# mfkiwl/conan-slam

Measured on AMD Instinct MI355X. Metric: ekf_update_steps_per_sec, higher is better.
Workload: dtype f32

## Files before the change

conan_slam_amd/csrc/cslam_ekf.hip:

```cpp
#include <hip/hip_runtime.h>

#include <algorithm>
#include <atomic>
#include <cfloat>
#include <cmath>
#include <cstdint>
#include <cstdlib>
#include <new>
#include <string>
#include <thread>
#include <vector>

#include "cslam_common.hpp"
#include "device_owners.hpp"
#include "ekf_kernels.hpp"
#include "ekf_kernels_fast.hpp"
#include "ekf_landmark_kernels.hpp"
#include "ekf_lookahead.hpp"
#include "ekf_pgemm_limbs.hpp"
#include "ekf_pose_kernels.hpp"
#include "host_linalg.hpp"

namespace cslam
{
__global__ void ekf_la_signal_kernel(unsigned* signal, unsigned add)
{
    if (threadIdx.x == 0)
    {
        atomicAdd(signal, add);
    }
}
__global__ void __launch_bounds__(128) ekf_la_wide_f32(LaWideArgs a)
{
    ekf_la_wide_body<1, 0>(a);
}
__global__ void __launch_bounds__(128) ekf_la_wide_f32_k64(LaWideArgs a)
{
    ekf_la_wide_body<1, 64>(a);
}
}

using namespace cslam;

namespace
{

std::atomic<int>& g_engines = ::cslam::live_engines();

constexpr int    kStagingSlots = 64;
constexpr size_t kLdsBudget    = 150 * 1024;

struct EkfBase
{
    virtual ~EkfBase() {}
    int         dtype    = CSLAM_F32;
    int         fuse_f64 = 1;
    int         pgemm_limbs_req = -1, limbs_kmin_req = -1;
    int         xcd_queues_req = -1;
    int         device   = 0;
    int         quirks   = CSLAM_Q_REF_EXACT;
    int         nmax     = 0;
    int         ncap     = 0;
    int         ldp      = 0;
    int         n        = 3;
    int         sync_mode = 1;
    int         seq_defer     = 1;
    int         lower         = 0;
    int         pipeline      = 0;
    int         pgemm_spare   = 16;
    int         gather_corr_wide = 1;
    int         pgemm_wgs     = 0;
    int         lookahead     = -1;
    Stream      stream_own, stream_b_own, stream_f_own;
    hipStream_t stream   = nullptr;
    hipStream_t stream_b = nullptr;
    long long   la_windows = 0;

    virtual int init()                                                                        = 0;
    virtual int set_state(const void* X, int n, const void* P, int ldp)                        = 0;
    virtual int get_state(void* X, void* P, int ldp)                                           = 0;
    virtual int get_x(void* X, int cap)                                                        = 0;
    virtual int get_landmarks(int first, int count, void* x, void* pll, void* pvl)             = 0;
    virtual int trace(double* tr)                                                              = 0;
    virtual int predict(double v, double swa, const void* Q, double wb, double dt)             = 0;
    virtual int update(const void* Z, int m, const void* R, const int* idf, int batch, bool on_device) = 0;
    virtual int augment(const void* Z, int q, const void* R)                                   = 0;
    virtual int observe_heading(double phi, int use)                                           = 0;
    virtual int associate(const void* Z, int m, const void* R, double g1, double g2, int* idf_out, int* kind) = 0;
    virtual int factor_status(int* flags, int clear)                                           = 0;
    virtual int set_profiling(int on)                                                          = 0;
    virtual int get_stage_times(double* ms, int* launches)                                     = 0;
    virtual int debug_last_update(void* PHT, void* S, void* G, void* W1, void* V, int* k)      = 0;
    virtual int set_deferred(int max_cols)                                                     = 0;
    virtual int do_flush()                                                                     = 0;
    virtual int resolve_predict()                                                              = 0;
    virtual void set_fuse_predict(int on)                                                      = 0;
    virtual int sync_all()                                                                     = 0;
    virtual int la_drain()                                                                     = 0;
};

template <typename T>
struct Ekf : EkfBase
{
    DevBuf<T>   dX, dP;
    DevBuf<T>   dPv;
    DevBuf<int> dPoseDone;
    DevBuf<int> dSign;
    DevBuf<T>   dLm;
    int  hd_cols[2] = {0, 0};
// ... 42 lines not shown
    DevBuf<unsigned char>    dStage;
    Event                    stage_ev[kStagingSlots];
    int         stage_next = 0;
    DevBuf<int> dTicket;
    int        pgemm_limbs = 0;
    int        xcd_queues  = 0;
    int        limbs_kmin  = 65;
    DevBuf<uint4> dWb;
    size_t        wb_bytes = 0;
    DevBuf<int2>  dTilesM;
    DevBuf<int>   dSegOff;
    DevBuf<int>   dTicketX;
    int        tilesM_built = 0;
    int        limb_parity = 0;
    unsigned   launch_parity = 0;
    int        psym_nt = -1;
    DevBuf<int2> dTiles;
    int   tiles_built = 0;
    int   n_sym_tiles = 0;
    int   num_cus     = 256;
    int sticky_host = 0;
    int last_k      = 0;
    int kp_call_limit = 0;
    int                     profiling = 0;
    unsigned                prof_count = 0;
    bool                    prof_sampled = false;
    std::vector<Event>      ev_pool;
    std::vector<int>        ev_stage;
    size_t                  ev_used = 0;

    ~Ekf() override
    {
        (void)hipSetDevice(device);
        if (stream)
        {
            (void)hipStreamSynchronize(stream);
        }
        if (stream_b && stream_b != stream)
        {
            (void)hipStreamSynchronize(stream_b);
        }
        if (stream_f)
        {
            (void)hipStreamSynchronize(stream_f);
        }
    }

    T* wbase(int region) const { return dW1.get() + (size_t)region * wcap * ldp; }

    int use_device() { CSLAM_HIP_TRY(hipSetDevice(device)); return CSLAM_OK; }

    int init() override
    {
        int rc = use_device();
        if (rc)
        {
            return rc;
        }
        if (xcd_queues_req >= 0)
        {
            xcd_queues = xcd_queues_req;
        }
        if (pgemm_limbs_req >= 0)
        {
            pgemm_limbs = (pgemm_limbs_req == 6 || pgemm_limbs_req == 9) ? pgemm_limbs_req : 0;
        }
// ... 30 lines not shown
        if ((rc = dX.alloc_zeroed((size_t)ldp, stream)) || (rc = dP.alloc_zeroed((size_t)ldp * ldp, stream)) ||
            (rc = dPv.alloc_zeroed((size_t)3 * ldp, stream)) || (rc = dPoseDone.alloc_zeroed(4, stream)) ||
            (rc = dFlags.alloc_zeroed(2, stream)) || (rc = hFlags.alloc(2)) ||
            (rc = dHead.alloc_zeroed((size_t)3 * ldp + 2, stream)))
        {
            return rc;
        }
        CSLAM_HIP_TRY(hipFuncSetAttribute(reinterpret_cast<const void*>(&ekf_factor_kernel<T>),
                                          hipFuncAttributeMaxDynamicSharedMemorySize, 160 * 1024));
        if (sizeof(T) == 4)
        {
            CSLAM_HIP_TRY(hipFuncSetAttribute(reinterpret_cast<const void*>(&ekf_factor_mfma_big_f32<128>),
                                              hipFuncAttributeMaxDynamicSharedMemorySize, 160 * 1024));
        }
        else
        {
            CSLAM_HIP_TRY(hipFuncSetAttribute(reinterpret_cast<const void*>(&ekf_factor_mfma_f64<64>),
                                              hipFuncAttributeMaxDynamicSharedMemorySize, 160 * 1024));
            CSLAM_HIP_TRY(hipFuncSetAttribute(reinterpret_cast<const void*>(&ekf_factor_mfma_f64<32>),
                                              hipFuncAttributeMaxDynamicSharedMemorySize, 160 * 1024));
            CSLAM_HIP_TRY(hipFuncSetAttribute(reinterpret_cast<const void*>(&ekf_downdate_f64<4>),
                                              hipFuncAttributeMaxDynamicSharedMemorySize, 160 * 1024));
            CSLAM_HIP_TRY(hipFuncSetAttribute(reinterpret_cast<const void*>(&ekf_downdate_f64<2>),
                                              hipFuncAttributeMaxDynamicSharedMemorySize, 160 * 1024));
        }
        CSLAM_TRY(dTicket.alloc_zeroed(2, stream));
        if (const char* sv = getenv("CSLAM_LA_K64"))
        {
            la_k64 = atoi(sv) ? 1 : 0;
        }
        if (const char* sv = getenv("CSLAM_LA_WG_SIGNAL"))
        {
            la_wg_signal = atoi(sv) ? 1 : 0;
        }
        if (const char* sv = getenv("CSLAM_PSYM_NT"))
        {
            psym_nt = atoi(sv) ? 1 : 0;
        }
        rc = ensure_k(64);
        if (rc)
        {
            return rc;
        }
        rc = ensure_w(128);
        if (rc)
        {
            return rc;
        }
        rc = ensure_m(64);
        if (rc)
        {
            return rc;
        }
        CSLAM_HIP_TRY(hipStreamSynchronize(stream));
        return CSLAM_OK;
    }

    int ensure_k(int k)
    {
        if (k <= kcap)
        {
            return CSLAM_OK;
        }
        int newk = round_up(std::max(k, 2 * kcap), 8);
        CSLAM_HIP_TRY(hipStreamSynchronize(stream));
        Workspace nw;
// ... 189 lines not shown
    {
        return sizeof(T) == 4 && (k8 <= 128 || limbs_take(k8)) && lower && ldp < 32768;
    }
    bool limbs_take(int k8) const
    {
        return sizeof(T) == 4 && pgemm_limbs > 0 && k8 >= limbs_kmin && k8 <= 256 && lower && ldp < 32768;
    }

    int launch_negcol_fix(T* W, int kcols, hipStream_t st)
    {
        const int tiles = round_up(n, kTile) / kTile;
        int       rc    = CSLAM_OK;
        if (lower && (rc = ensure_tile_list(tiles)))
        {
            return rc;
        }
        const int nt = lower ? n_sym_tiles : tiles * tiles;
        hipLaunchKernelGGL(ekf_negcol_fix_kernel<T>, dim3(std::min(nt, 2 * num_cus)), dim3(256), 0, st, dP.get(), ldp,
                           n, W, ldp, kcols, dSign.get() + (size_t)wcur * wcap, dSign.get() + (size_t)2 * wcap + wcur,
                           lower ? dTiles.get() : (const int2*)nullptr, nt, tiles, dPoseDone.get() + 2,
                           (stream_b == stream) ? 1 : 0);
        CSLAM_HIP_TRY(hipGetLastError());
        return CSLAM_OK;
    }

    int flush_wait()
    {
        int rc = flush();
        return rc ? rc : wait_pgemm();
    }

    size_t slot_bytes(int mc) const { return (size_t)mc * (2 * sizeof(T) + sizeof(int)); }

    int ensure_m(int m)
    {
        if (m <= mcap)
        {
            return CSLAM_OK;
        }
        int newm = std::max(m, 2 * mcap);
        if (int rc = la_drain())
        {
            return rc;
        }
        CSLAM_HIP_TRY(hipStreamSynchronize(stream));
        if (stream_f)
        {
            CSLAM_HIP_TRY(hipStreamSynchronize(stream_f));
        }
        PinnedBuf<unsigned char> hs;
        DevBuf<unsigned char>    ds;
        int                      rc = hs.alloc(slot_bytes(newm) * kStagingSlots);
        if (rc || (rc = ds.alloc(slot_bytes(newm) * kStagingSlots)))
        {
            return rc;
        }
        hStage = std::move(hs);
        dStage = std::move(ds);
        mcap = newm;
        return CSLAM_OK;
    }

    int stage_obs(const void* Z, const int* idf, int m, bool on_device, const T** dZ, const int** dIdf)
    {
        int rc = ensure_m(m);
        if (rc)
        {
            return rc;
        }
        int slot = stage_next;
        stage_next = (stage_next + 1) % kStagingSlots;
        if (stage_ev[slot])
        {
            CSLAM_HIP_TRY(hipEventSynchronize(stage_ev[slot].get()));
        }
        else if ((rc = stage_ev[slot].create(hipEventDisableTiming)))
        {
            return rc;
        }
        size_t         zb = (size_t)m * 2 * sizeof(T);
        unsigned char* ds = dStage.get() + slot_bytes(mcap) * slot;
        if (on_device)
        {
            hipLaunchKernelGGL(ekf_stage_obs_kernel<T>, dim3((3 * m + 255) / 256), dim3(256), 0, stream,
                               static_cast<const T*>(Z), idf, m, reinterpret_cast<T*>(ds), reinterpret_cast<int*>(ds + zb));
            CSLAM_HIP_TRY(hipGetLastError());
        }
        else
        {
            unsigned char* hs = hStage.get() + slot_bytes(mcap) * slot;
            memcpy(hs, Z, zb);
            memcpy(hs + zb, idf, (size_t)m * sizeof(int));
            CSLAM_HIP_TRY(hipMemcpyAsync(ds, hs, zb + (size_t)m * sizeof(int), hipMemcpyHostToDevice, stream));
        }
        CSLAM_HIP_TRY(hipEventRecord(stage_ev[slot].get(), stream));
        *dZ   = reinterpret_cast<const T*>(ds);
        *dIdf = reinterpret_cast<const int*>(ds + zb);
        return CSLAM_OK;
    }

    int set_state(const void* X, int nn, const void* P, int ldph) override
    {
        if (!X || !P || nn < 3 || nn > ncap || ((nn - 3) & 1) || ldph < nn)
        {
            return fail(CSLAM_ERR_BAD_ARG, "set_state: bad n=%d (cap %d) or ldp=%d", nn, ncap, ldph);
        }
        int rc = sync_all();
        if (rc)
        {
            return rc;
        }
        CSLAM_HIP_TRY(hipMemcpyAsync(dX.get(), X, (size_t)nn * sizeof(T), hipMemcpyHostToDevice, stream));
        CSLAM_HIP_TRY(hipMemcpy2DAsync(dP.get(), (size_t)ldp * sizeof(T), P, (size_t)ldph * sizeof(T),
                                       (size_t)nn * sizeof(T), (size_t)nn, hipMemcpyHostToDevice, stream));
        CSLAM_HIP_TRY(hipMemcpyAsync(dPv.get(), dP.get(), (size_t)3 * ldp * sizeof(T), hipMemcpyDeviceToDevice,
                                     stream));
        kp        = 0;
        wcur      = 0;
        last_slot = nullptr;
// ... 714 lines not shown
            if ((rc = launch_downdate(last_slot, k, stream)))
            {
                return rc;
            }
        }
        CSLAM_HIP_TRY(hipStreamSynchronize(stream));
        return CSLAM_OK;
    }


    struct LaUpd
    {
        const T*       dZ;
        const int*     dIdf;
        int            m;
        T              R[4];
        PredictArgs<T> pp;
    };
    struct FactorOut
    {
        DevBuf<T>   S, G, Gt, V, t, U, M, sub, xloc;
        DevBuf<int> idloc;
    };
    struct LaSet
    {
        Event          ev_fb;
        Event          ev_raw;
        FactorOut      fo[2];
        DevBuf<T>      XL, PvL, PH, PvLb, Dbb;
        DevBuf<T>      Y;
        DevBuf<LaModel<T>> model;
        DevBuf<unsigned>   done;
        DevBuf<long long>  stamps;
    };
    LaUpd       la_q[2];
    int         la_n = 0;
    LaSet       la;
    bool        la_ready = false;
    hipStream_t stream_f = nullptr;
    DevBuf<T>   la_WR;
    int         la_kpad  = 0;
    int         la_cus = 0;
    unsigned    la_target = 0;
    unsigned    la_seq    = 0;
    unsigned    la_sig_add = 0;
    int         la_k64 = 1;
    int         la_wg_signal = 0;

    int         la_fused   = 1;
    const T *dbgS = nullptr, *dbgGt = nullptr, *dbgV = nullptr;

    int la_ensure(int kp_cols)
    {
        constexpr int KM = 2 * kLaMaxObs;
        if (!la_ready)
        {
            int lo = 0, hi = 0;
            CSLAM_HIP_TRY(hipDeviceGetStreamPriorityRange(&lo, &hi));
            Stream sf;
            LaSet  nl;
            int    rc = sf.create_with_priority(hipStreamNonBlocking, hi);
            if (rc || (rc = nl.ev_fb.create(hipEventDisableTiming)) || (rc = nl.ev_raw.create(hipEventDisableTiming)))
            {
                return rc;
            }
            CSLAM_HIP_TRY(hipFuncSetAttribute(reinterpret_cast<const void*>(&ekf_la_chain_kernel<T, 32>),
                                              hipFuncAttributeMaxDynamicSharedMemorySize, (int)la_chain_lds<T>(32)));
            CSLAM_HIP_TRY(hipFuncSetAttribute(reinterpret_cast<const void*>(&ekf_la_chain_kernel<T, 64>),
                                              hipFuncAttributeMaxDynamicSharedMemorySize, (int)la_chain_lds<T>(64)));
            CSLAM_TRY(nl.done.alloc_zeroed_blocking(768));
            for (FactorOut& f : nl.fo)
            {
                const size_t kk = (size_t)KM * (KM + 1);
                if ((rc = f.S.alloc(kk)) || (rc = f.G.alloc(kk)) || (rc = f.Gt.alloc(kk)) || (rc = f.V.alloc(KM)) ||
                    (rc = f.t.alloc(KM)) || (rc = f.U.alloc(KM)) || (rc = f.M.alloc((size_t)3 * KM)) ||
                    (rc = f.sub.alloc((size_t)(3 + KM) * KM)) || (rc = f.xloc.alloc(3 + KM)) ||
                    (rc = f.idloc.alloc(kLaMaxObs)))
                {
                    return rc;
                }
            }
            if ((rc = nl.XL.alloc((size_t)2 * KM)) || (rc = nl.PvL.alloc((size_t)2 * KM * 3)) ||
                (rc = nl.PH.alloc((size_t)KM * KM)) || (rc = nl.PvLb.alloc((size_t)KM * 3)) ||
                (rc = nl.Dbb.alloc((size_t)KM * KM)) || (rc = nl.Y.alloc((size_t)KM * KM)) ||
                (rc = nl.model.alloc(2)) || (getenv("CSLAM_LA_STAMPS") && (rc = nl.stamps.alloc_zeroed_blocking(32))))
            {
                return rc;
            }
            if (const char* fv = getenv("CSLAM_LA_FUSED"))
            {
                la_fused = atoi(fv) ? 1 : 0;
            }
            stream_f_own = std::move(sf);
            stream_f     = stream_f_own.get();
            la           = std::move(nl);
            la_cus       = 1;
            la_target    = 0;
            la_seq       = 0;
            la_ready     = true;
        }
        if (kp_cols > la_kpad)
        {
            CSLAM_HIP_TRY(hipStreamSynchronize(stream));
            CSLAM_HIP_TRY(hipStreamSynchronize(stream_f));
            const int kpad = round_up(std::max(kp_cols, 128), 64);
            DevBuf<T> wr;
            CSLAM_TRY(wr.alloc((size_t)2 * KM * kpad));
            la_WR   = std::move(wr);
            la_kpad = kpad;
        }
        return CSLAM_OK;
    }

    bool la_eligible(int m) const
    {
        const int k = 2 * m;
        const bool on = lookahead > 0 || (lookahead < 0 && sizeof(T) == 4 && n >= 7000 && g_engines.load() == 1);
        return on && !sync_mode && !pipeline && profiling != 1 && k > 16 && k <= 2 * kLaMaxObs && gather_corr_wide &&
               fuse_predict && (sizeof(T) == 4 || fuse_f64) && defer_max >= k + (la_n ? 2 * la_q[0].m : k) &&
               wcap >= k + (la_n ? 2 * la_q[0].m : k) && seq.count == 0 && hd_cols[0] == 0 && hd_cols[1] == 0 && n > 3 &&
               kp_call_limit == 0;
    }

    int la_enqueue(const T* dZ, const int* dIdf, int m, const T* R, bool on_device)
    {
        if (on_device && la_n == 0)
        {
            if (int rc = stage_obs(dZ, dIdf, m, true, &dZ, &dIdf))
            {
                return rc;
            }
        }
        LaUpd u;
        u.dZ   = dZ;
        u.dIdf = dIdf;
        u.m    = m;
        for (int i = 0; i < 4; i++)
        {
            u.R[i] = R[i];
        }
        u.pp     = pp;
        pp.valid = 0;
        la_q[la_n++] = u;
        return la_n == 2 ? la_launch_window() : CSLAM_OK;
    }

    FactorArgs<T> la_factor_args(const LaUpd& u, FactorOut& f)
    {
        FactorArgs<T> a;
        a.X   = f.xloc.get();
        a.n   = 3 + 2 * u.m;
        a.Z   = u.dZ;
        a.idf = la.fo[0].idloc.get();
        a.m   = u.m;
        for (int i = 0; i < 4; i++)
        {
            a.R[i] = u.R[i];
        }
        a.PHT      = ws.dPHT.get();
        a.ldw      = ldp;
        a.dS       = f.S.get();
        a.dG       = f.G.get();
        a.dGt      = f.Gt.get();
        a.dV       = f.V.get();
        a.dt       = f.t.get();
        a.flags    = dFlags.get();
        a.scratchS = ws.dScrS.get();
        a.scratchG = ws.dScrG.get();
        a.textbook = (quirks & CSLAM_Q_LOWER_CHOL_GAIN) ? 0 : 1;
        a.stamps   = (la.stamps.get() && &f == &la.fo[0]) ? la.stamps.get() : nullptr;
        a.sub      = f.sub.get();
        a.dM       = f.M.get();
        a.pp       = PredictArgs<T>{0, (T)0, (T)0, (T)0, (T)0, (T)0, (T)0, (T)0, (T)0, 0};
        a.P3       = dPv.get();
        a.ldp3     = ldp;
        a.pred_out = nullptr;
        a.lds_S    = 1;
// ... 23 lines not shown
                               dX.get(), dP.get(), dPv.get(), ldp, n, u.dZ, u.dIdf, u.m, ws.dPHT.get(), ldp, lower,
                               (T*)nullptr, pa, pred, Wg, ldp, kp, (const int*)nullptr, dFlags.get(), (T*)nullptr);
        }
        else
        {
            const dim3 ggrid((n + 255) / 256, (u.m + kGatherObs - 1) / kGatherObs);
            hipLaunchKernelGGL(ekf_gather_kernel<T>, ggrid, dim3(256), 0, stream, dX.get(), dP.get(), dPv.get(), ldp, n,
                               u.dZ, u.dIdf, u.m, ws.dPHT.get(), ldp, lower, (T*)nullptr, pa, pred, Wg, ldp, kp,
                               (const int*)nullptr, dFlags.get(), (T*)nullptr);
        }
        CSLAM_HIP_TRY(hipGetLastError());
        if (ev_factor != nullptr)
        {
            CSLAM_HIP_TRY(hipStreamWaitEvent(stream, ev_factor, 0));
        }
        T*  slot = wbase(wcur) + (size_t)kp * ldp;
        rc       = launch_gain(k, slot, f.Gt.get(), f.U.get(), f.M.get());
        if (rc)
        {
            return rc;
        }
        pp.valid  = 0;
        fuse_now  = false;
        last_slot = slot;
        kp += k;
        dbgS      = f.S.get();
        dbgGt     = f.Gt.get();
        dbgV      = f.V.get();
        g_from_gt = true;
        sub_valid = false;
        return CSLAM_OK;
    }

    int la_launch_window()
    {
        const int nu = la_n;
        if (nu == 0)
        {
            return CSLAM_OK;
        }
        la_n = 0;
        const LaUpd ua = la_q[0], ub = la_q[1];
        const PredictArgs<T> held = pp;
        int rc = use_device();
        if (rc)
        {
            return rc;
        }
        const int ka = 2 * ua.m, kb = nu == 2 ? 2 * ub.m : 0;
        if (kp > 256 && (rc = flush()))
        {
            return rc;
        }
        if ((rc = ensure_k(2 * kLaMaxObs)) || (rc = ensure_w(ka + kb)) || (rc = la_ensure(kp)))
        {
            return rc;
        }
        if (lower && (rc = ensure_tile_list(round_up(n, kTile) / kTile)))
        {
            return rc;
        }
        const bool     safe     = g_engines.load() > 1;
        const unsigned n_blocks = (unsigned)(3 + ka + 2 * kb);
        auto launch_chain = [&]() -> int {
            LaChainArgs<T> ch;
            ch.fa   = la_factor_args(ua, la.fo[0]);
            ch.fb   = la_factor_args(nu == 2 ? ub : ua, la.fo[1]);
            ch.du_a = la.fo[0].U.get();
            ch.du_b = la.fo[1].U.get();
            ch.nu   = nu;
            ch.done = la.done.get();
            ch.target  = la_target + n_blocks;
            ch.timeout = 20000000ull;
            ch.chain_done = la.done.get() + 256;
            ch.seq        = ++la_seq;
            LaCarryArgs<T>& ca = ch.ca;
            ca.n       = n;
            ca.m_a     = ua.m;
            ca.m_b     = nu == 2 ? ub.m : 0;
            ca.idf_b   = nu == 2 ? ub.dIdf : ua.dIdf;
            ca.pp_b    = nu == 2 ? ub.pp : ua.pp;
            ca.PH      = la.PH.get();
            ca.Dbb     = la.Dbb.get();
            ca.PvLb    = la.PvLb.get();
            ca.XLb     = la.XL.get() + ka;
            ca.model_a = la.model.get();
            ca.Gt_a    = la.fo[0].Gt.get();
            ca.u_a     = la.fo[0].U.get();
            ca.M_a     = la.fo[0].M.get();
            ca.sub_a   = la.fo[0].sub.get();
            ca.sub_b   = la.fo[1].sub.get();
            ca.xloc_b  = la.fo[1].xloc.get();
            ca.model_b = la.model.get() + 1;
            ca.Y_b     = la.Y.get();
            if (std::max(ka, kb) <= 32)
            {
                hipLaunchKernelGGL((ekf_la_chain_kernel<T, 32>), dim3(1), dim3(256), la_chain_lds<T>(32), stream_f, ch);
            }
            else
            {
                hipLaunchKernelGGL((ekf_la_chain_kernel<T, 64>), dim3(1), dim3(256), la_chain_lds<T>(64), stream_f, ch);
            }
            CSLAM_HIP_TRY(hipGetLastError());
            CSLAM_HIP_TRY(hipEventRecord(la.ev_fb.get(), stream_f));
            return CSLAM_OK;
        };
        if (!safe && (rc = launch_chain()))
        {
            return rc;
        }
        const T* Wp = wbase(wcur);
        LaRowsArgs<T> ra;
        ra.X     = dX.get();
        ra.Pv    = dPv.get();
        ra.ldp   = ldp;
        ra.n     = n;
        ra.idf_a = ua.dIdf;
        ra.ra    = ka;
        ra.idf_b = nu == 2 ? ub.dIdf : ua.dIdf;
        ra.rb    = kb;
        ra.Wp    = Wp;
        ra.ldw   = ldp;
        ra.kp    = kp;
        ra.kpad  = la_kpad;
        ra.XL    = la.XL.get();
        ra.PvL   = la.PvL.get();
        ra.WR    = la_WR.get();
        ra.flags = dFlags.get();
        hipLaunchKernelGGL(ekf_la_rows_kernel<T>, dim3(ka + kb), dim3(128), 0, stream, ra);
        LaPrepArgs<T> pa;
        pa.P       = dP.get();
        pa.ldp     = ldp;
        pa.n       = n;
        pa.lower   = lower;
        pa.X       = dX.get();
        pa.Pv      = dPv.get();
        pa.idf_a   = ua.dIdf;
        pa.idf_b   = nu == 2 ? ub.dIdf : ua.dIdf;
        pa.ra      = ka;
        pa.rb      = kb;
        pa.pp_a    = ua.pp;
        pa.XL      = la.XL.get();
        pa.PvL     = la.PvL.get();
        pa.WR      = la_WR.get();
        pa.kp      = kp;
        pa.kpad    = la_kpad;
        pa.sub_a   = la.fo[0].sub.get();
        pa.PH      = la.PH.get();
        pa.Dbb     = la.Dbb.get();
        pa.PvLb    = la.PvLb.get();
        pa.model_a = la.model.get();
        pa.xloc_a  = la.fo[0].xloc.get();
        pa.idloc   = la.fo[0].idloc.get();
        const int  k8f      = round_up(kp, 8);
        const bool pg_signal = !la_wg_signal && !safe && kp > 0 && seq.count == 0 && sizeof(T) == 4 && k8f <= 128 && lower && ldp < 32768 &&
                               !limbs_take(k8f) && stream_b == stream && hd_cols[wcur] == 0;
        pa.done    = pg_signal ? (unsigned*)nullptr : la.done.get();
        hipLaunchKernelGGL(ekf_la_blocks_kernel<T>, dim3(n_blocks), dim3(64), 0, stream, pa);
        CSLAM_HIP_TRY(hipGetLastError());
        if (safe)
        {
            CSLAM_HIP_TRY(hipEventRecord(la.ev_raw.get(), stream));
            CSLAM_HIP_TRY(hipStreamWaitEvent(stream_f, la.ev_raw.get(), 0));
            if ((rc = launch_chain()))
            {
                return rc;
            }
        }
        la_target += n_blocks;
        la_sig_add = pg_signal ? n_blocks : 0u;
        rc         = flush();
        if (la_sig_add != 0)
        {
            const unsigned add = la_sig_add;
            la_sig_add         = 0;
            hipLaunchKernelGGL(ekf_la_signal_kernel, dim3(1), dim3(64), 0, stream, la.done.get(), add);
        }
        if (rc)
        {
            return rc;
        }
        bool fused = false;
        if constexpr (std::is_same<T, float>::value)
        {
            if (la_fused)
            {
                fused = true;
                if (safe)
                {
                    CSLAM_HIP_TRY(hipStreamWaitEvent(stream, la.ev_fb.get(), 0));
                }
                LaWideArgs wa;
                wa.chain_done = la.done.get() + 256;
                wa.seq        = la_seq;
                wa.timeout    = 20000000ull;
                wa.flags      = dFlags.get();
                wa.stamps     = la.stamps.get() ? la.stamps.get() + 16 : nullptr;
                wa.wg_times   = nullptr;
                wa.P       = dP.get();
                wa.ldp     = ldp;
                wa.n       = n;
                wa.lower   = getenv("CSLAM_LA_TIMING_DIRECT") ? 0 : lower;
                wa.X       = dX.get();
                wa.Pv      = dPv.get();
                wa.nu      = nu;
                wa.idf_a   = ua.dIdf;
                wa.idf_b   = nu == 2 ? ub.dIdf : ua.dIdf;
                wa.ma      = ua.m;
                wa.mb      = nu == 2 ? ub.m : 0;
                wa.valid_a = ua.pp.valid;
                wa.valid_b = nu == 2 ? ub.pp.valid : 0;
                wa.w_a     = ua.pp.w;
                wa.w_b     = nu == 2 ? ub.pp.w : 0;
                wa.model_a = la.model.get();
                wa.model_b = la.model.get() + 1;
                wa.Gt_a    = la.fo[0].Gt.get();
                wa.u_a     = la.fo[0].U.get();
                wa.M_a     = la.fo[0].M.get();
                wa.sub_a   = la.fo[0].sub.get();
                wa.Gt_b    = la.fo[1].Gt.get();
                wa.u_b     = la.fo[1].U.get();
                wa.M_b     = la.fo[1].M.get();
                wa.sub_b   = la.fo[1].sub.get();
                wa.Y_b     = la.Y.get();
                wa.W1a     = wbase(wcur) + (size_t)kp * ldp;
                wa.W1b     = wa.W1a + (size_t)ka * ldp;
                wa.ldw     = ldp;
                wa.wv_out  = ws.dWv.get();
                if (la_k64 && ua.m == 32 && (nu == 1 || ub.m == 32))
                {
                    hipLaunchKernelGGL(ekf_la_wide_f32_k64, dim3(round_up(n, kTile) / 32), dim3(128), 0, stream, wa);
                }
                else
                {
                    hipLaunchKernelGGL(ekf_la_wide_f32, dim3(round_up(n, kTile) / 32), dim3(128), 0, stream, wa);
                }
                CSLAM_HIP_TRY(hipGetLastError());
                last_slot = nullptr;
                last_k    = 0;
                kp += ka + kb;
                sub_valid = false;
            }
        }
        if (!fused && ((rc = la_wide(ua, la.fo[0], la.ev_fb.get())) || (nu == 2 && (rc = la_wide(ub, la.fo[1],
                                                                                                 nullptr)))))
        {
            return rc;
        }
        pp = held;
        la_windows++;
        if (la.stamps.get() && la_windows == 300)
        {
            long long h[32];
            CSLAM_HIP_TRY(hipStreamSynchronize(stream));
            CSLAM_HIP_TRY(hipMemcpy(h, la.stamps.get(), sizeof(h), hipMemcpyDeviceToHost));
            fprintf(stderr, "[cslam la wide stamps, 10 ns ticks] ids+columns issue:%lld poll+DMA wait:%lld pht_a:%lld gain_a:%lld store+share W1_a:%lld pht_b+corr:%lld share+G_b:%lld gain_b:%lld store_b:%lld\n",
                    h[17] - h[16], h[18] - h[17], h[19] - h[18], h[20] - h[19], h[21] - h[20], h[22] - h[21], h[23] - h[22],
                    h[24] - h[23], h[25] - h[24]);
            fprintf(stderr, "[cslam la stamps, cycles] load+observe:%lld sums:%lld symmetrise:%lld cholesky:%lld (first half %lld) inverse:%lld outputs:%lld total:%lld\n",
                    h[6] - h[0], h[7] - h[6], h[1] - h[7], h[2] - h[1], h[5] ? h[5] - h[1] : 0, h[3] - h[2], h[4] - h[3], h[4] - h[0]);
        }
        return CSLAM_OK;
    }

    int la_drain() override { return la_n ? la_launch_window() : CSLAM_OK; }

    int update(const void* Zv, int m, const void* Rv, const int* idf, int batch, bool on_device) override
    {
        if (m < 0 || !Rv || (m > 0 && (!Zv || !idf)))
        {
            return fail(CSLAM_ERR_BAD_ARG, "update: bad arguments (m=%d)", m);
        }
        if (m == 0)
        {
            return CSLAM_OK;
        }
        int rc = use_device();
        if (rc)
        {
            return rc;
        }
        const T*   R    = static_cast<const T*>(Rv);
        const T*   dZ   = static_cast<const T*>(Zv);
        const int* dIdf = idf;
        if (!on_device)
        {
            const int nf = (n - 3) / 2;
            for (int i = 0; i < m; i++)
            {
                if (idf[i] < 1 || idf[i] > nf)
                {
                    return fail(CSLAM_ERR_BAD_ARG, "update: idf[%d]=%d outside 1..%d", i, idf[i], nf);
                }
            }
            if ((rc = stage_obs(Zv, idf, m, false, &dZ, &dIdf)))
            {
                return rc;
            }
        }
        if (batch && la_eligible(m))
        {
            return la_enqueue(dZ, dIdf, m, R, on_device);
        }
        if ((rc = la_drain()))
        {
            return rc;
        }
        if (batch)
        {
            return batch_on_device(dZ, dIdf, m, R, false);
        }
        if ((rc = resolve_predict()))
        {
            return rc;
        }
        if (seq_defer)
        {
            if ((rc = ensure_w(2 * m + 8)))
            {
                return rc;
            }
            if (kp + 2 * m + 6 > wcap && (rc = flush()))
            {
                return rc;
            }
        }
        kp_call_limit = seq_defer ? kp + 2 * m : 0;
        for (int i = 0; i < m; i++)
// ... 699 lines not shown
        return rc;
    }
    return B(h)->associate(Z, m, R, gate1, gate2, idf_out, kind_out);
}

int cslam_ekf_observe_heading(cslam_ekf_t h, double phi, int use_heading)
{
    CSLAM_NEED(h);
    return B(h)->observe_heading(phi, use_heading);
}

int cslam_ekf_set_pgemm_workgroups(cslam_ekf_t h, int workgroups)
{
    CSLAM_NEED(h);
    if (workgroups < 0)
    {
        return fail(CSLAM_ERR_BAD_ARG, "set_pgemm_workgroups: negative");
    }
    B(h)->pgemm_wgs = workgroups;
    return CSLAM_OK;
}

int cslam_ekf_lookahead_windows(cslam_ekf_t h, long long* windows)
{
    CSLAM_NEED(h);
    if (!windows)
    {
        return fail(CSLAM_ERR_BAD_ARG, "lookahead_windows: null");
    }
    *windows = B(h)->la_windows;
    return CSLAM_OK;
}

int cslam_ekf_get_streams(cslam_ekf_t h, void** chain_stream, void** pgemm_stream)
{
    CSLAM_NEED(h);
    if (chain_stream)
    {
        *chain_stream = reinterpret_cast<void*>(B(h)->stream);
    }
    if (pgemm_stream)
    {
        *pgemm_stream = reinterpret_cast<void*>(B(h)->stream_b);
    }
    return CSLAM_OK;
}

int cslam_ekf_run_many(cslam_ekf_t* handles, int count, int steps, const double* v, const double* swa, const void* Q,
                       double wb, double dt, const void* const* dZ, const int* const* d_idf, int m, const void* R,
                       int batch)
{
    if (!handles || count < 0 || steps < 0 || m < 0 || !R || !Q || (steps > 0 && (!v || !swa)) || (m > 0 && (!dZ || !d_idf)))
    {
        return fail(CSLAM_ERR_BAD_ARG, "run_many: bad arguments");
    }
    for (int i = 0; i < count; i++)
    {
        if (!handles[i] || (m > 0 && (!dZ[i] || !d_idf[i])))
        {
            return fail(CSLAM_ERR_BAD_ARG, "run_many: null handle or input for instance %d", i);
        }
    }
    std::vector<int>         rcs((size_t)count, CSLAM_OK);
    std::vector<std::string> msgs((size_t)count);
    auto                     body = [&](int i) {
        EkfBase*     e     = B(handles[i]);
// ... 88 lines not shown
```

conan_slam_amd/csrc/ekf_lookahead.hpp:

```cpp
#pragma once

#include <hip/hip_runtime.h>

#include "ekf_kernels.hpp"
#include "ekf_kernels_fast.hpp"

namespace cslam
{

constexpr int kLaMaxObs = 32;

__device__ inline int la_row(const int* __restrict__ idf, int s, int n)
{
    return 3 + 2 * clamp_idf(idf[s >> 1], n) - 2 + (s & 1);
}

template <typename T>
struct LaRowsArgs
{
    const T* X;
    const T* Pv;
    int      ldp, n;
    const int* idf_a;
    int        ra;
    const int* idf_b;
    int        rb;
    const T*   Wp;
    int        ldw, kp, kpad;
    T *        XL, *PvL, *WR;
    int*       flags;
};

template <typename T>
__device__ __forceinline__ void ekf_la_rows_body(const LaRowsArgs<T>& a)
{
    const T* __restrict__ X = a.X;
    const T* __restrict__ Pv = a.Pv;
    const int ldp = a.ldp, n = a.n, ra = a.ra, rb = a.rb, ldw = a.ldw, kp = a.kp;
    const int* __restrict__ idf_a = a.idf_a;
    const int* __restrict__ idf_b = a.idf_b;
    const T* __restrict__ Wp = a.Wp;
    T* __restrict__ XL = a.XL;
    T* __restrict__ PvL = a.PvL;
    T* __restrict__ WR = a.WR;
    int* __restrict__ flags = a.flags;

    const int s   = blockIdx.x;
    if (threadIdx.x == 4)
    {
        const int id = (s < ra) ? idf_a[s >> 1] : idf_b[(s - ra) >> 1];
        if (id < 1 || id > ((n - 3) >> 1))
        {
            atomicOr(&flags[0], kFlagBadIdf);
        }
    }
    const int row = (s < ra) ? la_row(idf_a, s, n) : la_row(idf_b, s - ra, n);
    for (int q = threadIdx.x; q < kp; q += 128)
    {
        WR[(size_t)q * 128 + s] = Wp[(size_t)q * ldw + row];
    }
    if (threadIdx.x < 3)
    {
        PvL[s * 3 + threadIdx.x] = Pv[(size_t)threadIdx.x * ldp + row];
    }
    if (threadIdx.x == 3)
    {
        XL[s] = X[row];
    }
}

template <typename T>
__global__ void __launch_bounds__(128) ekf_la_rows_kernel(LaRowsArgs<T> a)
{
    ekf_la_rows_body<T>(a);
}


template <typename T>
struct LaModel
{
    T g02, g12;
    T pose[3];
    T pvv[9];
    T coef[kLaMaxObs * 10];
    T pad[2];
};

template <typename T>
__device__ inline void la_predict_row(const PredictArgs<T>& pp, T g02, T g12, int row, T* a)
{
    if (pp.valid && row - 3 < pp.w)
    {
        T o0, o1, o2;
        predict_stripe_col<T>(g02, g12, a[0], a[1], a[2], &o0, &o1, &o2);
        a[0] = o0;
        a[1] = o1;
        a[2] = o2;
    }
}

template <typename T>
__device__ inline void la_predict_pose(const PredictArgs<T>& pp, const T* pose_in, const T* pvv_in, T* pose, T* g, T* pvv)
{
    pose[0] = pose_in[0], pose[1] = pose_in[1], pose[2] = pose_in[2];
    g[0] = g[1] = (T)0;
    for (int e = 0; e < 9; e++)
// ... 622 lines not shown
        ekf_factor_mfma_f64_body<K>(a.fa, a.du_a);
    }
    if (a.nu == 2)
    {
        __builtin_amdgcn_fence(__ATOMIC_RELEASE, "workgroup");
        __syncthreads();
        __builtin_amdgcn_fence(__ATOMIC_ACQUIRE, "workgroup");
        ekf_la_carry_body<T>(a.ca, la_chain_smem);
        __builtin_amdgcn_fence(__ATOMIC_RELEASE, "workgroup");
        __syncthreads();
        __builtin_amdgcn_fence(__ATOMIC_ACQUIRE, "workgroup");
        if constexpr (std::is_same<T, float>::value)
        {
            ekf_factor_mfma_f32_body<K>(a.fb, a.du_b);
        }
        else
        {
            ekf_factor_mfma_f64_body<K>(a.fb, a.du_b);
        }
    }
    __builtin_amdgcn_fence(__ATOMIC_RELEASE, "agent");
    __syncthreads();
    if (threadIdx.x < 32)
    {
        __hip_atomic_store(a.chain_done + 16 * threadIdx.x, a.seq, __ATOMIC_RELAXED, __HIP_MEMORY_SCOPE_AGENT);
    }
}

template <typename T, int K>
__global__ void __launch_bounds__(256) ekf_la_chain_kernel(LaChainArgs<T> a)
{
    ekf_la_chain_body<T, K>(a);
}

struct LaWideArgs
{
    const float* P;
    int          ldp, n, lower;
    float*       X;
    float*       Pv;
    int          nu;
    const int *  idf_a, *idf_b;
    int          ma, mb;
    int          valid_a, valid_b, w_a, w_b;
    const LaModel<float>*model_a, *model_b;
    const float *Gt_a, *u_a, *M_a, *sub_a;
    const float *Gt_b, *u_b, *M_b, *sub_b, *Y_b;
    float *      W1a, *W1b;
    int          ldw;
    float*       wv_out;
    const unsigned* chain_done;
    unsigned        seq;
    unsigned long long timeout;
    int*            flags;
    long long*      stamps;
    long long*      wg_times;
};

__device__ __forceinline__ int la_q_of(int t, int r, int lh)
{
    return 32 * t + (r & 3) + 8 * (r >> 2) + 4 * lh;
}

template <int PAIRS = 1, int KFIX = 0>
__device__ __forceinline__ void ekf_la_wide_body(const LaWideArgs& a)
{
    __shared__ __attribute__((aligned(16))) float s_G[2][4 * 1024];
    __shared__ __attribute__((aligned(16))) float s_Y[4 * 1024];
    __shared__ __attribute__((aligned(16))) float s_model[2][512];
    __shared__ __attribute__((aligned(16))) float s_u[2][256];
    __shared__ __attribute__((aligned(16))) float s_M[2][256];
    __shared__ int   s_fx[2][kLaMaxObs];
    __shared__ float s_sum_all[PAIRS][4][32];
    const int tid = threadIdx.x, wave = __builtin_amdgcn_readfirstlane(tid >> 6), lane = tid & 63, lj = lane & 31, lh = lane >> 5;
    const int wv = wave & 1, pr = wave >> 1;
    float (*s_sum)[32] = s_sum_all[pr];
    const int row0 = (blockIdx.x * PAIRS + pr) * 32;
    const int row  = row0 + lj;
    const int rowc = row < a.n ? row : a.n - 1;
    const int ka = KFIX ? KFIX : 2 * a.ma, kb = KFIX ? KFIX : 2 * a.mb;
    int       stamp_i = 0;
    auto      stamp   = [&]() {
        if (a.stamps != nullptr && blockIdx.x == (gridDim.x >> 1) && tid == 0)
        {
            a.stamps[stamp_i++] = (long long)__builtin_amdgcn_s_memrealtime();
        }
    };
    stamp();
    if constexpr (PAIRS == 2)
// ... 556 lines not shown
```

conan_slam_amd/ekf.py:

```python
from __future__ import annotations

import ctypes as C

import numpy as np

from . import _capi
from ._capi import (F32, F64, Q_REF_EXACT, Q_TEXTBOOK, check)


def _vp(a: np.ndarray):
    return a.ctypes.data_as(C.c_void_p)


class EKF:
    def __init__(self, max_landmarks: int, dtype=np.float32, device: int = -1, quirks: int = Q_REF_EXACT,
                 sync_mode: bool = True):
        self.dtype = np.dtype(dtype)
        if self.dtype not in (np.dtype(np.float32), np.dtype(np.float64)):
            raise ValueError("dtype must be float32 or float64")
        self._L = _capi.lib()
        self._h = C.c_void_p(None)
        code = F32 if self.dtype == np.float32 else F64
        check(self._L.cslam_ekf_create(C.c_int(max_landmarks), C.c_int(code), C.c_int(device), C.c_int(quirks),
                                       C.byref(self._h)))
# ... 51 lines not shown
        assert P.shape == (n, n)
        check(self._L.cslam_ekf_set_state(self._h, _vp(X), C.c_int(n), _vp(P), C.c_int(n)))

    def get_state(self):
        n = self.n
        X = np.zeros(n, dtype=self.dtype)
        P = np.zeros((n, n), dtype=self.dtype, order="F")
        check(self._L.cslam_ekf_get_state(self._h, _vp(X), _vp(P), C.c_int(n)))
        return X, P

    def get_x(self):
        n = self.n
        X = np.zeros(n, dtype=self.dtype)
        check(self._L.cslam_ekf_get_x(self._h, _vp(X), C.c_int(n)))
        return X

    def get_p(self):
        return self.get_state()[1]

    X = property(get_x)
    P = property(get_p)

    def trace(self) -> float:
        t = C.c_double(0.0)
        check(self._L.cslam_ekf_trace(self._h, C.byref(t)))
        return t.value

    def synchronize(self):
        check(self._L.cslam_ekf_synchronize(self._h))

    def lookahead_windows(self) -> int:
        w = C.c_longlong(0)
        check(self._L.cslam_ekf_lookahead_windows(self._h, C.byref(w)))
        return w.value

    def landmarks(self, first: int = 1, count: int = None):
        if count is None:
            count = max((self.n - 3) // 2 - first + 1, 0)
        x = np.empty((count, 2), dtype=self.dtype)
        pll = np.empty((count, 4), dtype=self.dtype)
        pvl = np.empty((count, 6), dtype=self.dtype)
        check(self._L.cslam_ekf_get_landmarks(self._h, int(first), int(count), _vp(x), _vp(pll), _vp(pvl)))
        return x, pll.reshape(count, 2, 2).transpose(0, 2, 1).copy(), pvl.reshape(count, 2, 3).transpose(0, 2, 1).copy()

    def factor_status(self, clear: bool = False) -> int:
        f = C.c_int(0)
        check(self._L.cslam_ekf_factor_status(self._h, C.byref(f), C.c_int(1 if clear else 0)))
        return f.value

    def predict(self, v, swa, Q, wb, dt):
        Q = self._mat22(Q)
        check(self._L.cslam_ekf_predict(self._h, C.c_double(float(v)), C.c_double(float(swa)), _vp(Q),
                                        C.c_double(float(wb)), C.c_double(float(dt))))

    def update(self, Z, R, idf, batch: bool = False):
        Z = np.asarray(Z, dtype=self.dtype)
        m = 0 if Z.size == 0 else Z.reshape(2, -1, order="F").shape[1]
        Zc = self._arr(Z) if m else np.zeros(2, dtype=self.dtype)
        R = self._mat22(R)
        idf = np.ascontiguousarray(idf, dtype=np.int32)
        assert idf.shape[0] == m
        idp = idf.ctypes.data_as(C.c_void_p) if m else None
        check(self._L.cslam_ekf_update(self._h, _vp(Zc), C.c_int(m), _vp(R), idp, C.c_int(1 if batch else 0)))

    def update_device(self, dZ_ptr: int, m: int, R, d_idf_ptr: int, batch: bool = True):
        R = self._mat22(R)
# ... 221 lines not shown
```

include/cslam.h:

```cpp
#ifndef CSLAM_H
#define CSLAM_H

#ifdef __cplusplus
extern "C" {
#endif

#define CSLAM_VERSION 100

#define CSLAM_OK 0
#define CSLAM_ERR_BAD_ARG 1
#define CSLAM_ERR_CAPACITY 2
#define CSLAM_ERR_HIP 3
#define CSLAM_ERR_NO_DEVICE 4
#define CSLAM_ERR_ALLOC 5
#define CSLAM_FACTOR_OK 0
#define CSLAM_FACTOR_FALLBACK 1
#define CSLAM_FACTOR_ZEROED 2
#define CSLAM_FACTOR_SKIPPED 4
#define CSLAM_FACTOR_INTERNAL 16
#define CSLAM_FACTOR_BAD_IDF 8
#define CSLAM_FACTOR_HEADING_SKIPPED 32

#define CSLAM_F32 0
#define CSLAM_F64 1
// ... 19 lines not shown
int cslam_ekf_create(int max_landmarks, int dtype, int device, int quirks, cslam_ekf_t* out);
int cslam_ekf_destroy(cslam_ekf_t h);

int cslam_ekf_set_sync_mode(cslam_ekf_t h, int sync_mode);

int cslam_ekf_set_state(cslam_ekf_t h, const void* X, int n, const void* P, int ldp);
int cslam_ekf_get_state(cslam_ekf_t h, void* X, void* P, int ldp);
int cslam_ekf_get_x(cslam_ekf_t h, void* X, int capacity);
int cslam_ekf_get_n(cslam_ekf_t h, int* n);
int cslam_ekf_get_landmarks(cslam_ekf_t h, int first, int count, void* x, void* pll, void* pvl);
int cslam_ekf_trace(cslam_ekf_t h, double* trace);
int cslam_ekf_synchronize(cslam_ekf_t h);
int cslam_ekf_factor_status(cslam_ekf_t h, int* flags, int clear);

int cslam_ekf_predict(cslam_ekf_t h, double v, double swa, const void* Q, double wb, double dt);

int cslam_ekf_update(cslam_ekf_t h, const void* Z, int m, const void* R, const int* idf, int batch);

int cslam_ekf_update_device(cslam_ekf_t h, const void* dZ, int m, const void* R, const int* d_idf, int batch);

int cslam_ekf_augment(cslam_ekf_t h, const void* Z, int q, const void* R);

int cslam_ekf_observe_heading(cslam_ekf_t h, double phi, int use_heading);

int cslam_ekf_associate(cslam_ekf_t h, const void* Z, int m, const void* R, double gate1, double gate2, int* idf_out,
                        int* kind_out);

int cslam_ekf_set_deferred(cslam_ekf_t h, int max_pending_columns);
int cslam_ekf_flush(cslam_ekf_t h);

int cslam_ekf_get_streams(cslam_ekf_t h, void** chain_stream, void** pgemm_stream);

int cslam_ekf_lookahead_windows(cslam_ekf_t h, long long* windows);

int cslam_ekf_set_pgemm_workgroups(cslam_ekf_t h, int workgroups);

int cslam_ekf_run_many(cslam_ekf_t* handles, int count, int steps, const double* v, const double* swa, const void* Q,
                       double wb, double dt, const void* const* dZ, const int* const* d_idf, int m, const void* R,
                       int batch);

typedef struct cslam_ekf_batch* cslam_ekf_batch_t;
int cslam_ekf_batch_create(int instances, int n_landmarks, int device, int quirks, cslam_ekf_batch_t* out);
int cslam_ekf_batch_destroy(cslam_ekf_batch_t h);
int cslam_ekf_batch_set_state(cslam_ekf_batch_t h, int instance, const float* X, int n, const float* P, int ldp);
int cslam_ekf_batch_get_state(cslam_ekf_batch_t h, int instance, float* X, float* P, int ldp);
int cslam_ekf_batch_run(cslam_ekf_batch_t h, int steps, const double* v, const double* swa, const float* Q, double wb,
                        double dt, const float* const* dZ, const int* const* d_idf, int m, const float* R);
int cslam_ekf_batch_flush(cslam_ekf_batch_t h);
int cslam_ekf_batch_synchronize(cslam_ekf_batch_t h);
int cslam_ekf_batch_trace(cslam_ekf_batch_t h, double* traces );
int cslam_ekf_batch_factor_status(cslam_ekf_batch_t h, int* flags );
int cslam_ekf_batch_info(cslam_ekf_batch_t h, int* instances, int* n, long long* windows);
int cslam_ekf_batch_set_profiling(cslam_ekf_batch_t h, int every);
int cslam_ekf_batch_get_pgemm_time(cslam_ekf_batch_t h, double* ms_sum, int* launches);

int cslam_ekf_batch_create_capacity(int instances, int max_landmarks, int n_landmarks, int device, int quirks,
                                    cslam_ekf_batch_t* out);
int cslam_ekf_batch_predict(cslam_ekf_batch_t h, double v, double swa, const float* Q, double wb, double dt);
int cslam_ekf_batch_predict_each(cslam_ekf_batch_t h, const double* v, const double* swa, const float* Q, double wb,
                                 double dt);
int cslam_ekf_batch_get_poses(cslam_ekf_batch_t h, float* x, float* pvv);
int cslam_ekf_batch_get_landmarks(cslam_ekf_batch_t h, int first, int count, float* x, float* pll, float* pvl);
int cslam_ekf_batch_observe_heading(cslam_ekf_batch_t h, double phi, int use_heading);
int cslam_ekf_batch_update(cslam_ekf_batch_t h, const float* const* dZ, const int* const* d_idf, int m, const float* R);
int cslam_ekf_batch_augment(cslam_ekf_batch_t h, const float* const* dZn, int q, const float* R);

// ... 83 lines not shown
```

Baseline: 13190.

## Defer the lookahead wide kernel and fold next observation staging into it

The fused lookahead wide kernel launch is now held back until the next on-device update arrives. That update's Z/idf snapshot copy is then folded into the held launch as one extra block, which removes the separate stage_obs kernel launch per window. The rows kernel copies the second update's Z/idf into keep buffers, so the held wide kernel and the chain no longer depend on caller buffers that may be reused. This adds deferred-launch state that must be flushed on drain, on host updates and in the destructor, and it moves the cross-engine event wait into the held launch path.

```diff
diff --git a/conan_slam_amd/csrc/cslam_ekf.hip b/conan_slam_amd/csrc/cslam_ekf.hip
--- a/conan_slam_amd/csrc/cslam_ekf.hip
+++ b/conan_slam_amd/csrc/cslam_ekf.hip
@@ -30,12 +30,39 @@
         atomicAdd(signal, add);
     }
 }
+__device__ __forceinline__ bool la_wide_snapshot(const LaSnapJob& j)
+{
+    if (j.Z == nullptr || blockIdx.x + 1 != gridDim.x)
+    {
+        return false;
+    }
+    for (int i = threadIdx.x; i < 3 * j.m; i += 128)
+    {
+        if (i < 2 * j.m)
+        {
+            j.Z_out[i] = j.Z[i];
+        }
+        else
+        {
+            j.idf_out[i - 2 * j.m] = j.idf[i - 2 * j.m];
+        }
+    }
+    return true;
+}
 __global__ void __launch_bounds__(128) ekf_la_wide_f32(LaWideArgs a)
 {
+    if (la_wide_snapshot(a.snap))
+    {
+        return;
+    }
     ekf_la_wide_body<1, 0>(a);
 }
 __global__ void __launch_bounds__(128) ekf_la_wide_f32_k64(LaWideArgs a)
 {
+    if (la_wide_snapshot(a.snap))
+    {
+        return;
+    }
     ekf_la_wide_body<1, 64>(a);
 }
 }
@@ -75,6 +102,7 @@
     hipStream_t stream   = nullptr;
     hipStream_t stream_b = nullptr;
     long long   la_windows = 0;
+    long long   stage_launches = 0;
 
     virtual int init()                                                                        = 0;
     virtual int set_state(const void* X, int n, const void* P, int ldp)                        = 0;
@@ -183,6 +211,7 @@
     ~Ekf() override
     {
         (void)hipSetDevice(device);
+        (void)la_launch_held_wide(nullptr);
         if (stream)
         {
             (void)hipStreamSynchronize(stream);
@@ -279,6 +308,10 @@
         if (const char* sv = getenv("CSLAM_LA_WG_SIGNAL"))
         {
             la_wg_signal = atoi(sv) ? 1 : 0;
+        }
+        if (const char* sv = getenv("CSLAM_LA_HOLD_WIDE"))
+        {
+            la_hold_wide = atoi(sv) ? 1 : 0;
         }
         if (const char* sv = getenv("CSLAM_PSYM_NT"))
         {
@@ -534,6 +567,13 @@
 
     size_t slot_bytes(int mc) const { return (size_t)mc * (2 * sizeof(T) + sizeof(int)); }
 
+    int stage_take_slot()
+    {
+        const int slot = stage_next;
+        stage_next     = (stage_next + 1) % kStagingSlots;
+        return slot;
+    }
+
     int ensure_m(int m)
     {
         if (m <= mcap)
@@ -570,8 +610,7 @@
         {
             return rc;
         }
-        int slot = stage_next;
-        stage_next = (stage_next + 1) % kStagingSlots;
+        int slot = stage_take_slot();
         if (stage_ev[slot])
         {
             CSLAM_HIP_TRY(hipEventSynchronize(stage_ev[slot].get()));
@@ -587,6 +626,7 @@
             hipLaunchKernelGGL(ekf_stage_obs_kernel<T>, dim3((3 * m + 255) / 256), dim3(256), 0, stream,
                                static_cast<const T*>(Z), idf, m, reinterpret_cast<T*>(ds), reinterpret_cast<int*>(ds + zb));
             CSLAM_HIP_TRY(hipGetLastError());
+            stage_launches++;
         }
         else
         {
@@ -1367,7 +1407,18 @@
         DevBuf<LaModel<T>> model;
         DevBuf<unsigned>   done;
         DevBuf<long long>  stamps;
+        DevBuf<int>        idf_keep;
+        DevBuf<T>          z_keep;
     };
+    struct LaHeld
+    {
+        bool       valid = false;
+        bool       k64   = false;
+        unsigned   grid  = 0;
+        LaWideArgs wa;
+    };
+    LaHeld      la_held;
+    int         la_hold_wide = 1;
     LaUpd       la_q[2];
     int         la_n = 0;
     LaSet       la;
@@ -1418,7 +1469,9 @@
             if ((rc = nl.XL.alloc((size_t)2 * KM)) || (rc = nl.PvL.alloc((size_t)2 * KM * 3)) ||
                 (rc = nl.PH.alloc((size_t)KM * KM)) || (rc = nl.PvLb.alloc((size_t)KM * 3)) ||
                 (rc = nl.Dbb.alloc((size_t)KM * KM)) || (rc = nl.Y.alloc((size_t)KM * KM)) ||
-                (rc = nl.model.alloc(2)) || (getenv("CSLAM_LA_STAMPS") && (rc = nl.stamps.alloc_zeroed_blocking(32))))
+                (rc = nl.model.alloc(2)) || (rc = nl.idf_keep.alloc(kLaMaxObs)) ||
+                (rc = nl.z_keep.alloc(2 * kLaMaxObs)) ||
+                (getenv("CSLAM_LA_STAMPS") && (rc = nl.stamps.alloc_zeroed_blocking(32))))
             {
                 return rc;
             }
@@ -1457,11 +1510,74 @@
                kp_call_limit == 0;
     }
 
+    int la_launch_held_wide(const LaSnapJob* job)
+    {
+        if (!la_held.valid)
+        {
+            return CSLAM_OK;
+        }
+        if constexpr (std::is_same<T, float>::value)
+        {
+            int rc = use_device();
+            if (rc)
+            {
+                return rc;
+            }
+            if (g_engines.load() > 1)
+            {
+                CSLAM_HIP_TRY(hipStreamWaitEvent(stream, la.ev_fb.get(), 0));
+            }
+            LaWideArgs& wa = la_held.wa;
+            unsigned    g  = la_held.grid;
+            if (job != nullptr)
+            {
+                wa.snap = *job;
+                g += 1;
+            }
+            if (la_held.k64)
+            {
+                hipLaunchKernelGGL(ekf_la_wide_f32_k64, dim3(g), dim3(128), 0, stream, wa);
+            }
+            else
+            {
+                hipLaunchKernelGGL(ekf_la_wide_f32, dim3(g), dim3(128), 0, stream, wa);
+            }
+            CSLAM_HIP_TRY(hipGetLastError());
+        }
+        la_held.valid = false;
+        return CSLAM_OK;
+    }
+
     int la_enqueue(const T* dZ, const int* dIdf, int m, const T* R, bool on_device)
     {
         if (on_device && la_n == 0)
         {
-            if (int rc = stage_obs(dZ, dIdf, m, true, &dZ, &dIdf))
+            int rc = la_held.valid ? ensure_m(m) : CSLAM_OK;
+            if (rc)
+            {
+                return rc;
+            }
+            if constexpr (std::is_same<T, float>::value)
+            {
+                if (la_held.valid)
+                {
+                    unsigned char* ds = dStage.get() + slot_bytes(mcap) * stage_take_slot();
+                    LaSnapJob      job;
+                    job.Z       = dZ;
+                    job.idf     = dIdf;
+                    job.Z_out   = reinterpret_cast<T*>(ds);
+                    job.idf_out = reinterpret_cast<int*>(ds + (size_t)m * 2 * sizeof(T));
+                    job.m       = m;
+                    if ((rc = la_launch_held_wide(&job)))
+                    {
+                        return rc;
+                    }
+                    dZ       = job.Z_out;
+                    dIdf     = job.idf_out;
+                    on_device = false;
+                }
+            }
+            if (on_device && (rc = stage_obs(dZ, dIdf, m, true, &dZ, &dIdf)))
             {
                 return rc;
             }
@@ -1477,7 +1593,7 @@
         u.pp     = pp;
         pp.valid = 0;
         la_q[la_n++] = u;
-        return la_n == 2 ? la_launch_window() : CSLAM_OK;
+        return la_n == 2 ? la_launch_window(true) : CSLAM_OK;
     }
 
     FactorArgs<T> la_factor_args(const LaUpd& u, FactorOut& f)
@@ -1567,7 +1683,7 @@
         return CSLAM_OK;
     }
 
-    int la_launch_window()
+    int la_launch_window(bool may_hold = false)
     {
         const int nu = la_n;
         if (nu == 0)
@@ -1597,10 +1713,16 @@
         }
         const bool     safe     = g_engines.load() > 1;
         const unsigned n_blocks = (unsigned)(3 + ka + 2 * kb);
+        const bool hold = may_hold && la_hold_wide && la_fused && !safe && nu == 2 && std::is_same<T, float>::value &&
+                          !la.stamps.get();
         auto launch_chain = [&]() -> int {
             LaChainArgs<T> ch;
             ch.fa   = la_factor_args(ua, la.fo[0]);
             ch.fb   = la_factor_args(nu == 2 ? ub : ua, la.fo[1]);
+            if (hold)
+            {
+                ch.fb.Z = la.z_keep.get();
+            }
             ch.du_a = la.fo[0].U.get();
             ch.du_b = la.fo[1].U.get();
             ch.nu   = nu;
@@ -1613,7 +1735,7 @@
             ca.n       = n;
             ca.m_a     = ua.m;
             ca.m_b     = nu == 2 ? ub.m : 0;
-            ca.idf_b   = nu == 2 ? ub.dIdf : ua.dIdf;
+            ca.idf_b   = hold ? la.idf_keep.get() : (nu == 2 ? ub.dIdf : ua.dIdf);
             ca.pp_b    = nu == 2 ? ub.pp : ua.pp;
             ca.PH      = la.PH.get();
             ca.Dbb     = la.Dbb.get();
@@ -1662,6 +1784,9 @@
         ra.PvL   = la.PvL.get();
         ra.WR    = la_WR.get();
         ra.flags = dFlags.get();
+        ra.idf_b_keep = hold ? la.idf_keep.get() : (int*)nullptr;
+        ra.Z_b        = ub.dZ;
+        ra.Z_b_keep   = hold ? la.z_keep.get() : (T*)nullptr;
         hipLaunchKernelGGL(ekf_la_rows_kernel<T>, dim3(ka + kb), dim3(128), 0, stream, ra);
         LaPrepArgs<T> pa;
         pa.P       = dP.get();
@@ -1721,10 +1846,6 @@
             if (la_fused)
             {
                 fused = true;
-                if (safe)
-                {
-                    CSLAM_HIP_TRY(hipStreamWaitEvent(stream, la.ev_fb.get(), 0));
-                }
                 LaWideArgs wa;
                 wa.chain_done = la.done.get() + 256;
                 wa.seq        = la_seq;
@@ -1740,7 +1861,7 @@
                 wa.Pv      = dPv.get();
                 wa.nu      = nu;
                 wa.idf_a   = ua.dIdf;
-                wa.idf_b   = nu == 2 ? ub.dIdf : ua.dIdf;
+                wa.idf_b   = hold ? la.idf_keep.get() : (nu == 2 ? ub.dIdf : ua.dIdf);
                 wa.ma      = ua.m;
                 wa.mb      = nu == 2 ? ub.m : 0;
                 wa.valid_a = ua.pp.valid;
@@ -1762,15 +1883,15 @@
                 wa.W1b     = wa.W1a + (size_t)ka * ldp;
                 wa.ldw     = ldp;
                 wa.wv_out  = ws.dWv.get();
-                if (la_k64 && ua.m == 32 && (nu == 1 || ub.m == 32))
+                wa.snap    = LaSnapJob{nullptr, nullptr, nullptr, nullptr, 0};
+                la_held.wa    = wa;
+                la_held.k64   = la_k64 && ua.m == 32 && (nu == 1 || ub.m == 32);
+                la_held.grid  = (unsigned)(round_up(n, kTile) / 32);
+                la_held.valid = true;
+                if (!hold && (rc = la_launch_held_wide(nullptr)))
                 {
-                    hipLaunchKernelGGL(ekf_la_wide_f32_k64, dim3(round_up(n, kTile) / 32), dim3(128), 0, stream, wa);
+                    return rc;
                 }
-                else
-                {
-                    hipLaunchKernelGGL(ekf_la_wide_f32, dim3(round_up(n, kTile) / 32), dim3(128), 0, stream, wa);
-                }
-                CSLAM_HIP_TRY(hipGetLastError());
                 last_slot = nullptr;
                 last_k    = 0;
                 kp += ka + kb;
@@ -1798,7 +1919,7 @@
         return CSLAM_OK;
     }
 
-    int la_drain() override { return la_n ? la_launch_window() : CSLAM_OK; }
+    int la_drain() override { return la_n ? la_launch_window() : la_launch_held_wide(nullptr); }
 
     int update(const void* Zv, int m, const void* Rv, const int* idf, int batch, bool on_device) override
     {
@@ -1828,7 +1949,7 @@
                     return fail(CSLAM_ERR_BAD_ARG, "update: idf[%d]=%d outside 1..%d", i, idf[i], nf);
                 }
             }
-            if ((rc = stage_obs(Zv, idf, m, false, &dZ, &dIdf)))
+            if ((rc = la_launch_held_wide(nullptr)) || (rc = stage_obs(Zv, idf, m, false, &dZ, &dIdf)))
             {
                 return rc;
             }
@@ -2594,6 +2715,17 @@
     return CSLAM_OK;
 }
 
+int cslam_ekf_stage_launches(cslam_ekf_t h, long long* launches)
+{
+    CSLAM_NEED(h);
+    if (!launches)
+    {
+        return fail(CSLAM_ERR_BAD_ARG, "stage_launches: null");
+    }
+    *launches = B(h)->stage_launches;
+    return CSLAM_OK;
+}
+
 int cslam_ekf_get_streams(cslam_ekf_t h, void** chain_stream, void** pgemm_stream)
 {
     CSLAM_NEED(h);
diff --git a/conan_slam_amd/csrc/ekf_lookahead.hpp b/conan_slam_amd/csrc/ekf_lookahead.hpp
--- a/conan_slam_amd/csrc/ekf_lookahead.hpp
+++ b/conan_slam_amd/csrc/ekf_lookahead.hpp
@@ -29,6 +29,9 @@
     int        ldw, kp, kpad;
     T *        XL, *PvL, *WR;
     int*       flags;
+    int*       idf_b_keep;
+    const T*   Z_b;
+    T*         Z_b_keep;
 };
 
 template <typename T>
@@ -72,6 +75,15 @@
 template <typename T>
 __global__ void __launch_bounds__(128) ekf_la_rows_kernel(LaRowsArgs<T> a)
 {
+    const int sb = (int)blockIdx.x - a.ra;
+    if (a.idf_b_keep != nullptr && sb >= 0 && threadIdx.x == 5)
+    {
+        a.Z_b_keep[sb] = a.Z_b[sb];
+        if ((sb & 1) == 0)
+        {
+            a.idf_b_keep[sb >> 1] = a.idf_b[sb >> 1];
+        }
+    }
     ekf_la_rows_body<T>(a);
 }
 
@@ -760,6 +772,15 @@
 {
     ekf_la_chain_body<T, K>(a);
 }
+
+struct LaSnapJob
+{
+    const float* Z;
+    const int*   idf;
+    float*       Z_out;
+    int*         idf_out;
+    int          m;
+};
 
 struct LaWideArgs
 {
@@ -783,6 +804,7 @@
     int*            flags;
     long long*      stamps;
     long long*      wg_times;
+    LaSnapJob       snap;
 };
 
 __device__ __forceinline__ int la_q_of(int t, int r, int lh)
diff --git a/conan_slam_amd/ekf.py b/conan_slam_amd/ekf.py
--- a/conan_slam_amd/ekf.py
+++ b/conan_slam_amd/ekf.py
@@ -107,6 +107,16 @@
     def lookahead_windows(self) -> int:
         w = C.c_longlong(0)
         check(self._L.cslam_ekf_lookahead_windows(self._h, C.byref(w)))
+        return w.value
+
+    def streams(self):
+        a, b = C.c_void_p(None), C.c_void_p(None)
+        check(self._L.cslam_ekf_get_streams(self._h, C.byref(a), C.byref(b)))
+        return a.value or 0, b.value or 0
+
+    def stage_launches(self) -> int:
+        w = C.c_longlong(0)
+        check(self._L.cslam_ekf_stage_launches(self._h, C.byref(w)))
         return w.value
 
     def landmarks(self, first: int = 1, count: int = None):
diff --git a/include/cslam.h b/include/cslam.h
--- a/include/cslam.h
+++ b/include/cslam.h
@@ -75,6 +75,8 @@
 int cslam_ekf_get_streams(cslam_ekf_t h, void** chain_stream, void** pgemm_stream);
 
 int cslam_ekf_lookahead_windows(cslam_ekf_t h, long long* windows);
+
+int cslam_ekf_stage_launches(cslam_ekf_t h, long long* launches);
 
 int cslam_ekf_set_pgemm_workgroups(cslam_ekf_t h, int workgroups);
 
```

Result: faster. 13620 (median of 6 runs) (+3.3%).
